# nh2/lz4-frame-conduit

Hardware: AMD Instinct MI355X
Metric: GiB/s end-to-end (compress+decompress), 4 MiB blocks, 1/2/4/8 GPUs vs liblz4 (higher is better)
Workload: dtype u8

## Files before the change

### lz4_frame_conduit_amd/csrc/encode.cuh

```cuda
#pragma once
#include <type_traits>
#include "common.cuh"

namespace lz4f {

constexpr uint32_t MFLIMIT = 12, LASTLIT = 5, MINMATCH = 4;
constexpr uint32_t ENC_POOL_SHORT = 0x200u;

struct ChunkInfo {
    uint32_t nrec;
    uint32_t first_lit;
    uint32_t tail_lit;
    uint32_t body_size;
    uint32_t carry_in;
    uint32_t flags;
    uint64_t out_off;
};

struct EncGeom {
    uint64_t src_size;
    uint64_t first_off;
    uint32_t write_endmark;
    uint32_t block_size;
    uint32_t chunk_size;
    uint32_t chunks_per_block;
    uint32_t n_blocks;
    uint32_t n_chunks;
    uint32_t linked;
    uint32_t block_checksum;
    uint32_t header_size;
    uint8_t  header[20];
    uint32_t max_rec_per_chunk;
    uint64_t rec_pool;
    uint32_t seed_stride;
    uint32_t tiles_per_wg;
    uint32_t e1_solo;
    uint32_t hc_attempts;
    uint32_t hc_lazy;
};

struct EncPlace {
    uint64_t bstart, bend_abs;
    uint64_t cs_abs, ce_abs;
    uint64_t low_abs;
    uint64_t rd_end;
};
__device__ __forceinline__ bool enc_place(const EncGeom& g, uint32_t chunk, EncPlace& pl)
{
    const uint32_t blk = chunk / g.chunks_per_block, cib = chunk % g.chunks_per_block;
    pl.bstart = g.first_off + (uint64_t)blk * g.block_size;
    pl.bend_abs = (pl.bstart + g.block_size < g.src_size) ? pl.bstart + g.block_size : g.src_size;
// ... 39 lines not shown
constexpr uint32_t E1_HASH_LOG = 13;
#ifndef E1_WAVES
#define E1_WAVES 16
#endif
#ifdef E1_DEBUG
#define E1DBG(...) __VA_ARGS__
#else
#define E1DBG(...)
#endif
#define E1_DBG_AT (((uint64_t)gridDim.x) * (2 * E1_NSLICE * E1_REC_PER_SLICE))
struct alignas(16) E1Shared {
    uint16_t table[1u << E1_HASH_LOG];
    uint8_t  tags[1u << E1_HASH_LOG];
    uint32_t s_end[2][E1_NSLICE];
    uint8_t  s_n[2][E1_NSLICE];
    uint32_t next, cov;
    uint32_t first;
    uint32_t cur[16];
    uint32_t pieces[2];
    uint32_t mode, hits;
    uint32_t tail_d[2];
    uint32_t idle[64];
    alignas(16) uint8_t ring[E1_RING + 16];
};
static_assert(sizeof(E1Shared) <= 163840, "one workgroup per CU");
static_assert(64 * E1_WAVES >= E1_NSLICE, "a thread per slice when the lists are merged");
#ifndef E1_GRAB
#define E1_GRAB 8
#endif
#ifndef E1_GRAB_D
#define E1_GRAB_D 1
#endif
#ifndef E1_DENSE_PASS
#define E1_DENSE_PASS 1
#endif
#ifndef E1_V2
// ... 31 lines not shown
#endif
#ifndef E1_STEP_HIT
#define E1_STEP_HIT 1
#endif
constexpr uint32_t E1_GRAB_SPARSE = E1_GRAB, E1_GRAB_DENSE = E1_GRAB_D, E1_PROBE_SLICES = 16, E1_DENSE_HITS = 24;
static_assert((E1_GRAB_SPARSE & (E1_GRAB_SPARSE - 1u)) == 0, "a long helping's size is a power of two: its claims are aligned by masking");

struct __attribute__((aligned(4))) e1_w2 { uint32_t a, b; };
struct __attribute__((aligned(4))) e1_w3 { uint32_t a, b, c; };
__device__ __forceinline__ uint32_t e1_ld32(const uint8_t* ring, uint32_t pos)
{
    const uint32_t i = pos & E1_RMASK;
    const e1_w2 w = *(const e1_w2*)(ring + (i & ~3u));
    return __builtin_amdgcn_alignbyte(w.b, w.a, i & 3u);
}
__device__ __forceinline__ uint64_t e1_ld64(const uint8_t* ring, uint32_t pos)
{
    const uint32_t i = pos & E1_RMASK;
    const e1_w3 w = *(const e1_w3*)(ring + (i & ~3u));
    return (uint64_t)__builtin_amdgcn_alignbyte(w.b, w.a, i & 3u) | ((uint64_t)__builtin_amdgcn_alignbyte(w.c, w.b, i & 3u) << 32);
}
#if E1_V7
static_assert(E1_ROWS >= 1 && E1_ROWS <= 8, "rows per round");
constexpr uint32_t E1_ROW_BYTES = 4 * 64, E1_ROUND_BYTES = E1_ROWS * E1_ROW_BYTES;
struct e1_rows { e1_w2 s1[E1_ROWS], s2[E1_ROWS]; };
__device__ __forceinline__ e1_rows e1_rows_ld(const uint8_t* ring, uint32_t base, uint32_t d, uint32_t lane)
{
    e1_rows w;
#pragma unroll
    for (uint32_t r = 0; r < E1_ROWS; r++) {
// ... 63 lines not shown
    t = (uint32_t)__builtin_amdgcn_update_dpp((int)v, (int)v, 0x112 , 0xf, 0xf, false); v = t < v ? t : v;
    t = (uint32_t)__builtin_amdgcn_update_dpp((int)v, (int)v, 0x114 , 0xf, 0xf, false); v = t < v ? t : v;
    t = (uint32_t)__builtin_amdgcn_update_dpp((int)v, (int)v, 0x118 , 0xf, 0xf, false); v = t < v ? t : v;
    return (uint32_t)__builtin_amdgcn_readlane((int)v, 15);
}
__device__ __forceinline__ uint32_t wave_excl_scan_max(uint32_t v)
{
    const uint32_t lane = lane_id();
    uint32_t incl = v;
#pragma unroll
    for (int sft = 1; sft < 64; sft <<= 1) { const uint32_t t = __shfl_up(incl, sft); if ((int)lane >= sft) incl = t > incl ? t : incl; }
    const uint32_t ex = __shfl_up(incl, 1);
    return lane == 0 ? 0u : ex;
}
constexpr uint32_t E1_PIECE_LOG = 12, E1_NPIECE = E1_TILE >> E1_PIECE_LOG;
__device__ __forceinline__ void e1_dma_piece(E1Shared& sh, const uint8_t* __restrict__ src, uint64_t org, uint32_t nts, uint32_t pc)
{
    const uint32_t lane = lane_id();
    const uint32_t ring0 = (uint32_t)(uintptr_t)(lptr_t)sh.ring;
#pragma unroll
    for (uint32_t q = 0; q < 4; q++) {
        const uint32_t at = nts + (pc << E1_PIECE_LOG) + q * 1024u;
        const uint8_t* gsrc = src + (org + at + lane * 16u);
        const uint32_t ldst = uni(ring0 + (at & E1_RMASK));
        uint32_t keep;
        asm volatile("s_mov_b32 %0, m0\n\ts_mov_b32 m0, %2\n\ts_nop 0\n\tglobal_load_lds_dwordx4 %1, off\n\ts_mov_b32 m0, %0" : "=&s"(keep) : "v"(gsrc), "s"(ldst) : "memory");
    }
}

__device__ __forceinline__ void e1_fill(E1Shared& sh, const uint8_t* __restrict__ src, uint64_t org, uint32_t a, uint32_t b, uint32_t tid)
// ... 142 lines not shown
                        le = st + ml;
                    }
                    cur = nx2;
                }
                const uint32_t e = (sj < nslice) ? s_end[sj] : 0u; cov = e > cov ? e : cov;
            }
        }
        ChunkInfo* ci = info + c;
        if (lane == 0) {
            if (room) { ci->nrec = ktot; ci->first_lit = tile_first; ci->tail_lit = te - kmax; ci->body_size = btot; }
            else      { ci->nrec = 0; ci->first_lit = 0; ci->tail_lit = te - ts; ci->body_size = 0; }
            sh.mode = (uint64_t)ktot * 64 > (uint64_t)(te - ts) ? 2u : 1u;
        }
    };

    if (tid == 0) { sh.mode = 0; sh.cov = E1_TILE; sh.hits = 0; sh.first = 0; sh.next = E1_ALIGN ? 0 : 1; sh.pieces[0] = 0; sh.pieces[1] = 0; sh.tail_d[0] = 0; sh.tail_d[1] = 0; }
    if (tid < 16) sh.cur[tid] = 0;
    uint32_t mode_tile = 0;
    uint32_t hold = 1;
    bool pend = false;
    uint32_t p_c = 0, p_par = 0, p_ts = 0, p_te = 0, p_bend = 0, p_ns = 0;
    __syncthreads();
    for (uint32_t c = c0; c < c1; c++) {
        const uint32_t k = c - c0;
        const uint32_t ts = E1_TILE * (k + 1), par = k & 1u;
        const uint32_t blk = c / g.chunks_per_block;
        const uint64_t bstart = g.first_off + (uint64_t)blk * g.block_size;
        const uint64_t bend_abs = (bstart + g.block_size < g.src_size) ? bstart + g.block_size : g.src_size;
        const uint64_t cs_abs = s0 + (uint64_t)k * E1_TILE;
        if (cs_abs >= bend_abs) {
            ChunkInfo* ci = info + c;
            if (tid == 0) { ci->nrec = 0; ci->first_lit = 0; ci->tail_lit = 0; ci->body_size = 0; }
            continue;
        }
        const uint32_t tlen = (uint32_t)((bend_abs - cs_abs < E1_TILE) ? bend_abs - cs_abs : E1_TILE);
        const uint32_t te = ts + tlen;
        const uint32_t bend = ts + (uint32_t)(bend_abs - cs_abs);
        const uint32_t blen = (uint32_t)(bend_abs - bstart);
        const uint32_t nslice = (tlen + E1_SLICE - 1) / E1_SLICE;
        uint32_t low = hist0;
// ... 1 lines not shown
        uint64_t* spec_t = spec + (size_t)par * (E1_NSLICE * E1_REC_PER_SLICE);

        uint32_t nlen = 0;
        const uint32_t nts = ts + E1_TILE;
        if (c + 1 < c1) {
            const uint32_t nblk = (c + 1) / g.chunks_per_block;
            const uint64_t nbstart = g.first_off + (uint64_t)nblk * g.block_size;
            const uint64_t nbend = (nbstart + g.block_size < g.src_size) ? nbstart + g.block_size : g.src_size;
            const uint64_t ncs = cs_abs + E1_TILE;
            if (ncs < nbend) nlen = (uint32_t)((nbend - ncs < E1_TILE) ? nbend - ncs : E1_TILE);
        }
        const bool nlen_full = nlen == E1_TILE;

        E1DBG(const unsigned long long q0 = clock64();)
        if (pend && wave == E1_WAVES - 1) {
            *(lane == 0 ? &sh.cur[wave] : &sh.idle[lane]) = 0xFFFFFFFFu;
            merge(p_c, p_par, p_ts, p_te, p_bend, p_ns);
        }

        E1DBG(const unsigned long long q1 = clock64();)
        const uint32_t end_lim = (te < bend - LASTLIT) ? te : bend - LASTLIT;
        E1DBG(uint32_t dq = 0; unsigned long long a_deq = 0, a_probe = 0, a_hit = 0, n_step = 0, n_hit = 0, n_deq = 0;)
        bool fresh = true;
        E1DBG(unsigned long long z0 = 0;)
#if E1_V5
        const uint32_t lim_t = (!(g.e1_solo & 2u) && blen >= MFLIMIT + 1) ? ((te - MINMATCH < bend - MFLIMIT) ? te - MINMATCH : bend - MFLIMIT) : 0u;
        const bool tile_plain = !(E1_ALIGN && mode_tile == 1u && !(g.e1_solo & 1u));
        bool plain = tile_plain || hold;
#endif
        auto release = [&](const uint32_t si, const uint32_t grab) __attribute__((always_inline)) {
            if (nlen_full && (si & 31u) < grab) {
                uint32_t mn = lane < E1_WAVES ? __hip_atomic_load(&sh.cur[lane], __ATOMIC_RELAXED, __HIP_MEMORY_SCOPE_WORKGROUP) : 0xFFFFFFFFu;
                mn = wave_min16(mn);
                uint32_t ok_p = mn == 0xFFFFFFFFu ? 0u : (mn * E1_SLICE) >> E1_PIECE_LOG;
                if (ok_p > E1_NPIECE) ok_p = E1_NPIECE;
                const uint32_t had = uni(atomicMax(lane == 0 ? &sh.pieces[par] : &sh.idle[lane], ok_p));
                for (uint32_t pc = had; pc < ok_p; pc++) e1_dma_piece(sh, src, org, ts + E1_TILE, pc);
            }
        };
        auto helping = [&](const uint32_t si, uint32_t ip, const uint32_t mode, const uint32_t grab, const bool opener) __attribute__((always_inline)) {
            const uint32_t cs = ts + si * E1_SLICE;
            uint64_t* myrec = spec_t + si * E1_REC_PER_SLICE;
            E1DBG(a_deq += clock64() - z0;)
            uint32_t nrec = 0, anchor = cs;
            if (ip < cs) ip = cs;
#if E1_V5
            {
                uint32_t last_start = cs + grab * E1_SLICE - 1u;
                if (lim_t < last_start) last_start = lim_t;
#else
            const uint32_t ce = (cs + grab * E1_SLICE < te) ? cs + grab * E1_SLICE : te;
            if (!(g.e1_solo & 2u) && blen >= MFLIMIT + 1 && ip + MINMATCH <= te && ip + MFLIMIT <= bend && ip < ce) {
                uint32_t last_start = ce - 1;
                if (te - MINMATCH < last_start) last_start = te - MINMATCH;
                if (bend - MFLIMIT < last_start) last_start = bend - MFLIMIT;
#endif
                const uint32_t floor_b = ip;
                uint32_t step = (E1_STEP0 > 1 && mode == 1 && !opener) ? (uint32_t)E1_STEP0 : 1u, two = opener ? 0u : 1u;
                E1DBG(uint32_t it = 0;)
                while (ip <= last_start) {
                    E1DBG(if (++it > 100000) { if (lane == 0) { atomicAdd((unsigned long long*)&scratch[E1_DBG_AT + 1], 1ull); scratch[E1_DBG_AT + 8] = ((uint64_t)ip << 32) | last_start; scratch[E1_DBG_AT + 9] = ((uint64_t)step << 32) | si; } break; })
                    E1DBG(const unsigned long long z1 = clock64(); n_step++;)
                    const uint32_t ipB = ip + WAVE * step, stepB = step + 1;
                    const uint32_t pA = ip + lane * step, pB = ipB + lane * stepB;
                    const bool actA = pA <= last_start, actB = two && pB <= last_start;
#if E1_V3
                    const uint32_t iA = pA & E1_RMASK, iB = pB & E1_RMASK;
// ... 92 lines not shown
                            const uint32_t pe = dpp_excl_scan_max(is_t ? lane + fl : 0u);
                            const uint32_t before = pe ? ip + pe : anchor;
                            const uint32_t bfloor = pe ? ip + pe : (anchor > floor_b ? anchor : floor_b);
                            uint32_t nb = nbk;
                            if (pA - bfloor < nb) nb = pA - bfloor;
                            if (pA - di - low < nb) nb = pA - di - low;
                            const uint32_t rank = (uint32_t)__builtin_popcountll(taken & ((1ull << lane) - 1ull));
                            if (is_t) myrec[nrec + rank] = pack_rec(pA - nb - before, fl + nb, di);
                            nrec += (uint32_t)__builtin_popcountll(taken);
                            E1DBG(if (blockIdx.x == 0 && lane == 0) { atomicAdd((unsigned long long*)&scratch[E1_DBG_AT + 13], 1ull); atomicAdd((unsigned long long*)&scratch[E1_DBG_AT + 14], (unsigned long long)__builtin_popcountll(taken)); atomicAdd((unsigned long long*)&scratch[E1_DBG_AT + 15], (unsigned long long)(stop_at < WAVE ? stop_at : (endrel > WAVE ? endrel : WAVE))); })
                            anchor = ip + endrel;
                            const uint32_t nrel = stop_at < WAVE ? stop_at : (endrel > WAVE ? endrel : WAVE);
                            const bool ins2 = actA && lane > L && lane < nrel && lane >= pe;
                            *(ins2 ? &sh.table[hA] : (uint16_t*)&sh.idle[lane]) = (uint16_t)pA; *(ins2 ? &sh.tags[hA] : (uint8_t*)&sh.idle[lane]) = (uint8_t)tgA;
                            ip += nrel;
                            atomicMax(lane == 0 ? &sh.cov : &sh.idle[lane], anchor);
                            step = 1; two = 1;
                            E1DBG(a_hit += clock64() - z2;)
                            continue;
                        }
                    }
                    E1DBG(if (blockIdx.x == 0 && lane == 0) { atomicAdd((unsigned long long*)&scratch[E1_DBG_AT + 4 + (inB ? 0 : mode != 2 ? 1 : step != 1 ? 2 : 3)], 1ull); })
                    const uint32_t dsel = inB ? dB : dA;
                    uint32_t mp = (uint32_t)__builtin_amdgcn_readlane(inB ? pB : pA, L);
                    const uint32_t d = (uint32_t)__builtin_amdgcn_readlane(dsel, L);
                    uint32_t room = mp - (anchor > floor_b ? anchor : floor_b); if (mp - d - low < room) room = mp - d - low;
                    uint32_t nb = 0;
                    E1DBG(uint32_t itb = 0;)
#if E1_V4
                    uint32_t fw = 0;
                    {
// ... 21 lines not shown
                    }
#endif
                    for (bool more = nb == WAVE; more;) {
                        E1DBG(if (++itb > 100000) { if (lane == 0) { atomicAdd((unsigned long long*)&scratch[E1_DBG_AT + 2], 1ull); scratch[E1_DBG_AT + 10] = ((uint64_t)room << 32) | nb; } break; })
                        const uint32_t kb = nb + lane + 1;
                        const uint32_t b1 = sh.ring[(mp - kb) & E1_RMASK], b2 = sh.ring[(mp - d - kb) & E1_RMASK];
                        const uint64_t ne = __ballot(b1 != b2 || kb > room);
                        const uint32_t n1 = ne ? (uint32_t)__builtin_ctzll(ne) : WAVE;
                        nb += n1;
                        more = n1 == WAVE;
                    }
                    E1DBG(uint32_t itf = 0;)
                    while (fw >> 31) {
                        fw &= 0x7FFFFFFFu;
                        E1DBG(if (++itf > 100000) { if (lane == 0) { atomicAdd((unsigned long long*)&scratch[E1_DBG_AT + 3], 1ull); scratch[E1_DBG_AT + 11] = ((uint64_t)mp << 32) | fw; scratch[E1_DBG_AT + 12] = ((uint64_t)end_lim << 32) | d; } break; })
#if E1_V7
                        const uint32_t a0 = mp + fw;
                        const e1_rows w = e1_rows_ld(sh.ring, a0, d, lane);
                        const uint32_t n = e1_rows_same(w, a0 & 3u, (a0 - d) & 3u), cap = end_lim - mp;
                        fw += n;
                        fw = (n == E1_ROUND_BYTES && fw < cap) ? (fw | 0x80000000u) : (fw < cap ? fw : cap);
#else
                        const uint32_t a0 = mp + fw + lane * 16;
                        const e1_w5 s1 = e1_ld5(sh.ring, a0), s2 = e1_ld5(sh.ring, a0 - d);
                        uint32_t g0 = e1_same16(s1, s2, a0 & 3u, (a0 - d) & 3u);
                        const int32_t r = (int32_t)(end_lim - a0); g0 = r <= 0 ? 0u : (g0 > (uint32_t)r ? (uint32_t)r : g0);
                        const uint64_t stop = __ballot(g0 < 16);
                        if (stop) { const uint32_t f = (uint32_t)__builtin_ctzll(stop); fw += f * 16 + (uint32_t)__builtin_amdgcn_readlane(g0, f); }
                        else fw = (fw + WAVE * 16) | 0x80000000u;
#endif
                    }
#else
                    for (;;) {
                        E1DBG(if (++itb > 100000) { if (lane == 0) { atomicAdd((unsigned long long*)&scratch[E1_DBG_AT + 2], 1ull); scratch[E1_DBG_AT + 10] = ((uint64_t)room << 32) | nb; } break; })
                        const uint32_t kb = nb + lane + 1;
                        const bool eq = kb <= room && sh.ring[(mp - kb) & E1_RMASK] == sh.ring[(mp - d - kb) & E1_RMASK];
                        const uint64_t ne = __ballot(!eq);
                        const uint32_t n1 = ne ? (uint32_t)__builtin_ctzll(ne) : WAVE;
                        nb += n1;
                        if (n1 < WAVE) break;
                    }
                    uint32_t fw = 0;
                    E1DBG(uint32_t itf = 0;)
                    for (;;) {
                        E1DBG(if (++itf > 100000) { if (lane == 0) { atomicAdd((unsigned long long*)&scratch[E1_DBG_AT + 3], 1ull); scratch[E1_DBG_AT + 11] = ((uint64_t)mp << 32) | fw; scratch[E1_DBG_AT + 12] = ((uint64_t)end_lim << 32) | d; } break; })
                        const uint32_t a0 = mp + fw + lane * 8;
                        uint32_t g0 = 0;
                        if (a0 < end_lim) {
                            const uint64_t x = e1_ld64(sh.ring, a0) ^ e1_ld64(sh.ring, a0 - d);
                            g0 = x ? (uint32_t)(__builtin_ctzll(x) >> 3) : 8u;
                            const uint32_t r = end_lim - a0; if (g0 > r) g0 = r;
                        }
                        const uint64_t stop = __ballot(g0 < 8);
                        if (stop) { const uint32_t f = (uint32_t)__builtin_ctzll(stop); fw += f * 8 + (uint32_t)__builtin_amdgcn_readlane(g0, f); break; }
                        fw += WAVE * 8;
                    }
#endif
                    mp -= nb;
                    const uint32_t mlen = nb + fw;
                    myrec[nrec] = pack_rec(mp - anchor, mlen, d);
                    nrec++;
                    anchor = ip = mp + mlen;
                    step = (E1_STEP_HIT > 1 && mode == 1) ? (uint32_t)E1_STEP_HIT : 1u; two = 1;
                    atomicMax(lane == 0 ? &sh.cov : &sh.idle[lane], ip);
                    if (E1_OPENER == 2) *((lane == 0 && ip == end_lim) ? &sh.tail_d[par] : &sh.idle[lane]) = d;
                    E1DBG(a_hit += clock64() - z2;)
                    if (E1_IP2 && ip >= low + 2 && ip + 2 <= te) { const uint32_t q2 = ip - 2, hv2 = e1_mix(e1_ld32(sh.ring, q2)); *(lane == 0 ? &sh.table[e1_slot(hv2)] : (uint16_t*)&sh.idle[lane]) = (uint16_t)q2; *(lane == 0 ? &sh.tags[e1_slot(hv2)] : (uint8_t*)&sh.idle[lane]) = (uint8_t)e1_tag(hv2); }
                }
            }
            const bool mine_s = lane < grab && si + lane < nslice;
            *(mine_s ? &sh.s_end[par][si + lane] : &sh.idle[lane]) = (lane == 0 && nrec) ? anchor : 0u;
            *(mine_s ? &sh.s_n[par][si + lane] : (uint8_t*)&sh.idle[lane]) = (uint8_t)(lane == 0 ? nrec : 0u);
            if (mode == 0) atomicAdd(lane == 0 ? &sh.hits : &sh.idle[lane], nrec);
            if (opener) *(lane == 0 ? &sh.first : &sh.idle[lane]) = 1u;
        };
        for (;;) {
            if ((g.e1_solo & 1u) && tid >= WAVE) break;
            E1DBG(z0 = clock64(); n_deq++;)
            E1DBG(if (++dq > 100000) { if (lane == 0) atomicAdd((unsigned long long*)&scratch[E1_DBG_AT + 0], 1ull); break; })
#if E1_V5
            if (!plain) {
                const uint32_t a = atomicAdd(lane == 0 ? &sh.next : &sh.idle[lane], E1_GRAB_SPARSE);
                const uint32_t cv = __hip_atomic_load(&sh.cov, __ATOMIC_RELAXED, __HIP_MEMORY_SCOPE_WORKGROUP);
                __builtin_amdgcn_sched_barrier(0);
                const uint32_t si = uni(a);
                if (si >= nslice) { *(lane == 0 ? &sh.cur[wave] : &sh.idle[lane]) = 0xFFFFFFFFu; break; }
                *(lane == 0 ? &sh.cur[wave] : &sh.idle[lane]) = si;
                release(si, E1_GRAB_SPARSE);
                helping(si, uni(cv), 1u, E1_GRAB_SPARSE, false);
                continue;
            }
            plain = tile_plain;
#endif
            uint32_t mode = (g.e1_solo & 1u) ? mode_tile : uni(__hip_atomic_load(&sh.mode, __ATOMIC_RELAXED, __HIP_MEMORY_SCOPE_WORKGROUP));
            const bool opener = fresh && wave == 0 && (!E1_ALIGN || hold);
            uint32_t grab = opener ? 1u : mode == 1 ? E1_GRAB_SPARSE : mode == 2 ? E1_GRAB_DENSE : 1u;
            uint32_t si = 0;
            if (E1_ALIGN && opener) si = uni(atomicAdd(lane == 0 ? &sh.next : &sh.idle[lane], grab));
            if (!opener) {
                if (fresh && E1_OPENER && ((E1_OPENER == 1 && !E1_ALIGN) || hold)) for (uint32_t spin = 0; spin < 4096 && uni(__hip_atomic_load(&sh.first, __ATOMIC_RELAXED, __HIP_MEMORY_SCOPE_WORKGROUP)) == 0; spin++) __builtin_amdgcn_s_sleep(2);
                bool got = false;
#if E1_V6
                if (E1_ALIGN && mode == 1) {
                    uint32_t n = uni(__hip_atomic_load(&sh.next, __ATOMIC_RELAXED, __HIP_MEMORY_SCOPE_WORKGROUP));
                    for (uint32_t t = 0; t < 64 && !got; t++) {
                        const uint32_t tgt = (n & ~(E1_GRAB_SPARSE - 1u)) + E1_GRAB_SPARSE;
                        const uint32_t old = uni(atomicCAS(lane == 0 ? &sh.next : &sh.idle[lane], n, tgt));
                        if (old == n) { got = true; si = n; grab = tgt - n; }
                        n = old;
                    }
                }
#endif
                if (!got) si = uni(atomicAdd(lane == 0 ? &sh.next : &sh.idle[lane], grab));
            }
            fresh = false;
            if (si >= nslice) { *(lane == 0 ? &sh.cur[wave] : &sh.idle[lane]) = 0xFFFFFFFFu; break; }
            *(lane == 0 ? &sh.cur[wave] : &sh.idle[lane]) = si;
            release(si, grab);
            if (mode == 0 && si >= 2 * E1_PROBE_SLICES) {
                mode = uni(__hip_atomic_load(&sh.hits, __ATOMIC_RELAXED, __HIP_MEMORY_SCOPE_WORKGROUP)) > E1_DENSE_HITS ? 2u : 1u;
                *(lane == 0 ? &sh.mode : &sh.idle[lane]) = mode;
                mode_tile = mode;
            }
            helping(si, uni(__hip_atomic_load(&sh.cov, __ATOMIC_RELAXED, __HIP_MEMORY_SCOPE_WORKGROUP)), mode, grab, opener);
        }
        E1DBG(const unsigned long long q2 = clock64();)
        __builtin_amdgcn_s_waitcnt(0);
        __syncthreads();
        mode_tile = uni(__hip_atomic_load(&sh.mode, __ATOMIC_RELAXED, __HIP_MEMORY_SCOPE_WORKGROUP));
        E1DBG(const unsigned long long q3 = clock64();)
        pend = true; p_c = c; p_par = par; p_ts = ts; p_te = te; p_bend = bend; p_ns = nslice;

        if (tid == 0) { sh.tail_d[par ^ 1u] = 0; sh.cov = nts; sh.hits = 0; sh.first = 0; sh.next = E1_ALIGN ? 0 : 1; sh.pieces[par ^ 1u] = 0; }
        if (tid < 16) sh.cur[tid] = 0;
        if (nlen) {
            if (nlen_full) {
                const uint32_t had = sh.pieces[par];
                for (uint32_t pc = had + wave; pc < E1_NPIECE; pc += E1_WAVES) e1_dma_piece(sh, src, org, nts, pc);
                if ((nts & E1_RMASK) == 0 && tid >= 64 && tid < 68) ((uint32_t*)(sh.ring + E1_RING))[tid - 64] = *(const u32_ua*)(src + (org + nts + (tid - 64) * 4u));
            } else e1_fill(sh, src, org, nts, nts + nlen, tid);
        }
        E1DBG(const unsigned long long q4 = clock64();)
        asm volatile("s_waitcnt vmcnt(0)" ::: "memory");
        E1DBG(const unsigned long long q5 = clock64();)
        __syncthreads();
        {
            const uint32_t td = uni(__hip_atomic_load(&sh.tail_d[par], __ATOMIC_RELAXED, __HIP_MEMORY_SCOPE_WORKGROUP));
            hold = (g.e1_solo & 1u) || (td != 0 && nlen >= 4 && uni(e1_ld32(sh.ring, nts)) == uni(e1_ld32(sh.ring, nts - td))) ? 1u : 0u;
        }
        E1DBG(if (blockIdx.x == 0 && lane == 0) { unsigned long long* d = (unsigned long long*)&scratch[E1_DBG_AT + 16 + wave * 8]; d[0] += q1 - q0; d[1] += q2 - q1; d[2] += q3 - q2; d[3] += q4 - q3; d[4] += q5 - q4; d[5] += clock64() - q5; d[6] += 1; unsigned long long* f = (unsigned long long*)&scratch[E1_DBG_AT + 160 + wave * 6]; f[0] += a_deq; f[1] += a_probe; f[2] += a_hit; f[3] += n_deq; f[4] += n_step; f[5] += n_hit; })
    }
    if (pend && wave == E1_WAVES - 1) merge(p_c, p_par, p_ts, p_te, p_bend, p_ns);
}


__device__ __forceinline__ uint32_t layout_block_chunks(ChunkInfo* __restrict__ ci, const uint32_t nch, const uint32_t blen)
{
    const uint32_t lane = lane_id();
    uint32_t carry_run = 0, total = 0;
    for (uint32_t c0 = 0; c0 < nch; c0 += WAVE) {
        const uint32_t c = c0 + lane;
        const bool act = c < nch;
        const uint4 x = act ? *(const uint4*)&ci[c] : uint4{0u, 0u, 0u, 0u};
// ... 538 lines not shown
```

### lz4_frame_conduit_amd/csrc/engine.hip

```cpp
#include <hip/hip_runtime.h>
#include <stdarg.h>
#include <stdio.h>
#include <stdlib.h>
#include <string.h>

#include <algorithm>
#include <mutex>
#include <vector>

#include "engine.hpp"
#include "frame_dev.cuh"
#include "decode_batch.cuh"
#include "encode_batch.cuh"
#include "measure_batch.cuh"
#include "pack_batch.cuh"

using namespace lz4f;

static_assert(sizeof(ChunkInfo) == 32, "chunk info layout");
static_assert(sizeof(BatchFrame) == 80 && sizeof(BatchBlk) == 40, "batch workspace layout");
static_assert(sizeof(BatchCore) == 64 && sizeof(MeasBlk) == 24, "batch measure workspace layout");
static_assert(sizeof(BcFrame) == 72 && sizeof(BcBlk) == 32 && sizeof(BcChunk) == 64, "batch encode workspace layout");

namespace lz4f {
// ... 56 lines not shown
    no_density_probe = on("LZ4F_MI355X_NO_DENSITY_PROBE");
    no_spx = on("LZ4F_MI355X_NO_SPX");
    no_overlap = on("LZ4F_MI355X_NO_OVERLAP");
    no_content_check = on("LZ4F_MI355X_NO_CONTENT_CHECK");
    prof = on("LZ4F_MI355X_PROF");
    e1_sync = on("LZ4F_MI355X_E1_SYNC");
    no_selffeed = on("LZ4F_MI355X_NO_SELFFEED");
    dense_mode = (unsigned)num("LZ4F_MI355X_DENSE_MODE", 0, 2, 0);
    group_kib = (unsigned)num("LZ4F_MI355X_GROUP_KIB", 64, 4096, 0);
    if (group_kib & (group_kib - 1)) group_kib = 0;
    feed_round = (unsigned)num("LZ4F_MI355X_FEED_ROUND", 17, 4096, 0);
    chain_gate = num("LZ4F_MI355X_CHAIN_GATE", 1, (1 << 20) - 1, 0);
    decode_mode = 0; if (const char* v = getenv("LZ4F_MI355X_DECODE")) decode_mode = v[0];
    e1_run = (unsigned)num("LZ4F_MI355X_E1_RUN", 1, 4096, 0);
    e1_solo = 0; if (const char* v = getenv("LZ4F_MI355X_E1_SOLO")) e1_solo = (unsigned)atoi(v);
    if (on("LZ4F_MI355X_DETERMINISTIC")) e1_solo |= 1u;
    wait_ticks = 0; if (const char* v = getenv("LZ4F_MI355X_WAIT_TICKS")) { unsigned long long a = 0; if (sscanf(v, "%llu", &a) == 1) wait_ticks = a; }
    dblk_lds = (unsigned)num("LZ4F_MI355X_DBLK_LDS", 1, 150, 0) << 10;
    recs_per_tile = (unsigned)num("LZ4F_MI355X_RECS_PER_TILE", 1, 16385, 0);
    hc_attempts = (unsigned)num("LZ4F_MI355X_HC_ATTEMPTS", 1, 65536, 0);
    hc_lazy = (unsigned)num("LZ4F_MI355X_HC_LAZY", 1, 2, 0);
    seed = 2; if (const char* v = getenv("LZ4F_MI355X_SEED")) { unsigned a = 0; if (sscanf(v, "%u", &a) == 1 && a >= 1 && a <= 64) seed = a; }
}
namespace lz4f {
size_t new_engine(lz4f_mi355x_engine** out, int device, void* stream, bool borrow)
{
    int n = 0;
    hipError_t e = hipGetDeviceCount(&n);
    if (e != hipSuccess || n <= 0) {
        set_last_error("no usable HIP device (hipGetDeviceCount: %s, count %d): liblz4f_mi355x has no CPU fallback", hipGetErrorString(e), n);
// ... 169 lines not shown
    g.seed_stride = sw.seed;
    const bool hc = j.level >= 3;
    p.finder = hc ? EncodePlan::HASH_CHAIN : ((sw.e1_solo & 1u) && !(sw.e1_solo & 4u)) ? EncodePlan::E1_SOLO : EncodePlan::E1_SHARED;
    if (hc) {
        const HcLevel hl = hc_level(j.level);
        g.hc_attempts = sw.hc_attempts ? sw.hc_attempts : hl.attempts;
        g.hc_lazy = sw.hc_lazy ? sw.hc_lazy : hl.lazy;
    }
    g.rec_pool = rec_pool_records(g.n_chunks, g.max_rec_per_chunk, ((sw.e1_solo & 1u) || hc) ? 16385u : sw.recs_per_tile);
    if (g.n_chunks) {
        uint32_t run = g.n_chunks / cus; run = run < 1 ? 1 : run > 64 ? 64 : run;
        if ((g.n_chunks + run - 1) / run > 1024) run = (g.n_chunks + 1023) / 1024;
        if (sw.e1_run) run = sw.e1_run;
        g.tiles_per_wg = run;
        g.e1_solo = sw.e1_solo;
        p.e1_wgs = (g.n_chunks + run - 1) / run;
        p.e1_scratch_bytes = (size_t)p.e1_wgs * 2 * E1_NSLICE * E1_REC_PER_SLICE * 8 + 2048;
    }
    p.layout_small = g.n_blocks <= LAYOUT_SMALL_BLOCKS && g.n_chunks <= LAYOUT_SMALL_CHUNKS; p.e2_split = g.n_chunks <= 512;
    p.xxh_lane4 = g.n_blocks < XXH_LANE4_BELOW;
    p.inband = inband;
    p.index_cap = inband ? index_capacity(payload, s) + 64 : index_cap;
    p.ixtmp_bytes = inband ? p.index_cap + 64 : 0;
    p.info_bytes = (size_t)(g.n_chunks + 1) * sizeof(ChunkInfo); p.recs_bytes = (size_t)(rec_pool_at(g.n_chunks) + g.rec_pool) * 8;
    p.blk_bytes = (size_t)(g.n_blocks + 1) * 4; p.table_bytes = (size_t)(g.n_blocks + 1) * sizeof(BlockOut);
    p.res_bytes = sizeof(ResultRec) + sizeof(TrailerPlan) + 64;
    return p;
}

#ifdef E1_DEBUG
static void e1_debug_dump(hipStream_t st, const uint8_t* counters)
{
    unsigned long long d[256]; if (hipStreamSynchronize(st) == hipSuccess && hipMemcpy(d, counters, 2048, hipMemcpyDeviceToHost) == hipSuccess) {
                for (int w = 0; w < 16; w += 5) { unsigned long long* x = d + 16 + w * 8; if (x[6]) fprintf(stderr, "E1 wave %d: per tile cycles: merge %llu parse %llu waitB1 %llu dma-issue %llu dma-wait %llu waitB2 %llu (%llu tiles)\n", w, x[0]/x[6], x[1]/x[6], x[2]/x[6], x[3]/x[6], x[4]/x[6], x[5]/x[6], x[6]); unsigned long long* f = d + 160 + w * 6; fprintf(stderr, "   parse: dequeue %llu cycles x %llu, probe step %llu cycles x %llu, hit %llu cycles x %llu (per tile)\n", f[3] ? f[0]/f[3] : 0, f[3]/x[6], f[4] ? f[1]/f[4] : 0, f[4]/x[6], f[5] ? f[2]/f[5] : 0, f[5]/x[6]); }
                fprintf(stderr, "E1 dense passes (workgroup 0): %llu, matches taken %llu, positions advanced %llu; one-match steps because: hit in B %llu, mode not dense %llu, step != 1 %llu, first match long %llu\n", d[13], d[14], d[15], d[4], d[5], d[6], d[7]);
                fprintf(stderr, "E1 debug: bounds hit: dequeue %llu, probe %llu, backward %llu, forward %llu; probe ip/last %llx step/slice %llx; back room/nb %llx; fwd mp/fw %llx end_lim/d %llx\n", d[0], d[1], d[2], d[3], d[8], d[9], d[10], d[11], d[12]); }
}
#endif

size_t lz4f_mi355x_engine::enc_workspaces(const EncodePlan& p, bool own_table)
{
    if (ixtmp.ensure(p.ixtmp_bytes) || res.ensure(p.res_bytes) || info.ensure(p.info_bytes) || recs.ensure(p.recs_bytes) || blk_bytes.ensure(p.blk_bytes) ||
        (own_table && table.ensure(p.table_bytes)) || e1_scratch.ensure(p.e1_scratch_bytes))
        return make_err(LZ4F_ERROR_allocation_failed);
    return 0;
}

size_t lz4f_mi355x_engine::enc_find(const CompressJob& j, const EncodePlan& p)
{
    hipStream_t st = (hipStream_t)stream; const EncGeom& g = p.g;
#ifdef E1_DEBUG
// ... 1037 lines not shown
```

### lz4_frame_conduit_amd/csrc/engine.hpp

```cpp
#pragma once
#include <stddef.h>
#include <stdint.h>
#include <functional>
#include <string>
#include <vector>

#include "../../include/lz4f_mi355x.h"
#include "records.hpp"

namespace lz4f {

inline size_t make_err(int code) { return (size_t)-(ptrdiff_t)code; }
inline bool   is_err(size_t v) { return v > make_err(LZ4F_ERROR_maxCode); }
const char*   err_name(size_t v);
void          set_last_error(const char* fmt, ...);
const char*   last_error();

struct Xxh32State {
    uint32_t total_len, large, v[4], memsize;
    uint8_t  mem[16];
    void reset(uint32_t seed = 0);
    void update(const void* data, size_t len);
    uint32_t digest() const;
};
// ... 41 lines not shown
    lz4f::DevBuf pdbuf;
    lz4f::DevBuf tight;
    lz4f::DevBuf postab;
    lz4f::DevBuf desc, seqcnt;
    lz4f::DevBuf d_in, d_out;
    lz4f::DevBuf bframes, btable;
    lz4f::DevBuf mframes, mtable;
    lz4f::DevBuf pctl;
    lz4f::DevBuf cframes, cblocks, cchunks;
    lz4f::PinBuf h_in, h_out, h_small;
    struct Switches {
        bool no_index, no_selfindex, no_resolve, no_trace, no_doubling, trace_always, no_groups, no_window, serial_walk, no_trailer, no_content_check, no_density_probe, no_spx, no_overlap, prof, e1_sync, no_selffeed;
        unsigned dense_mode;
        unsigned group_kib;
        unsigned feed_round;
        int chain_gate; char decode_mode; unsigned e1_run, e1_solo, seed, dblk_lds, recs_per_tile, hc_attempts, hc_lazy; unsigned long long wait_ticks;
        void read();
    } sw;
    void*  recs_ctl_clean = nullptr;
    size_t ix_seq_cap = 0;
    bool  timing = false;
    void* ev[24] = {nullptr};
    bool  ev_used[12] = {false};
    void  tick(int slot, bool end, void* on_stream = nullptr);
    void* aux_stream = nullptr; void* ev_fork = nullptr; void* ev_join = nullptr;
    bool  aux_ready();
    bool  aux_pending = false;

    struct CompressJob {
        const uint8_t* d_src; uint64_t src_size; uint64_t first_off;
        uint32_t block_size; bool linked; bool block_checksum; bool endmark;
// ... 104 lines not shown
```

Baseline: 794.0.

## Replace end-of-tile barrier with per-piece landed bits so next tile starts early

```diff
diff --git a/lz4_frame_conduit_amd/csrc/encode.cuh b/lz4_frame_conduit_amd/csrc/encode.cuh
--- a/lz4_frame_conduit_amd/csrc/encode.cuh
+++ b/lz4_frame_conduit_amd/csrc/encode.cuh
@@ -35,6 +35,7 @@
     uint32_t seed_stride;
     uint32_t tiles_per_wg;
     uint32_t e1_solo;
+    uint32_t e1_close;
     uint32_t hc_attempts;
     uint32_t hc_lazy;
 };
@@ -104,12 +105,14 @@
     uint8_t  tags[1u << E1_HASH_LOG];
     uint32_t s_end[2][E1_NSLICE];
     uint8_t  s_n[2][E1_NSLICE];
-    uint32_t next, cov;
-    uint32_t first;
-    uint32_t cur[16];
-    uint32_t pieces[2];
-    uint32_t mode, hits;
-    uint32_t tail_d[2];
+    uint32_t next[2], cov[2];
+    uint32_t first[2];
+    uint32_t cur[2][16];
+    uint32_t hits[2];
+    uint32_t landed[2];
+    uint32_t pieces[4];
+    uint32_t mode;
+    uint32_t tail_d[4];
     uint32_t idle[64];
     alignas(16) uint8_t ring[E1_RING + 16];
 };
@@ -171,6 +174,12 @@
     const e1_w2 w = *(const e1_w2*)(ring + (i & ~3u));
     return __builtin_amdgcn_alignbyte(w.b, w.a, i & 3u);
 }
+__device__ __forceinline__ uint32_t e1_ld32_wrap(const uint8_t* ring, uint32_t pos)
+{
+    const uint32_t i = pos & E1_RMASK, i0 = i & ~3u;
+    const uint32_t a = *(const uint32_t*)(ring + i0), b = *(const uint32_t*)(ring + ((i0 + 4u) & E1_RMASK));
+    return __builtin_amdgcn_alignbyte(b, a, i & 3u);
+}
 __device__ __forceinline__ uint64_t e1_ld64(const uint8_t* ring, uint32_t pos)
 {
     const uint32_t i = pos & E1_RMASK;
@@ -264,6 +273,31 @@
     return lane == 0 ? 0u : ex;
 }
 constexpr uint32_t E1_PIECE_LOG = 12, E1_NPIECE = E1_TILE >> E1_PIECE_LOG;
+#if E1_V4 && E1_V7
+constexpr uint32_t E1_FWD_BYTES = E1_ROUND_BYTES;
+#elif E1_V4
+constexpr uint32_t E1_FWD_BYTES = 64 * 16;
+#else
+constexpr uint32_t E1_FWD_BYTES = 64 * 8;
+#endif
+constexpr uint32_t E1_REACH = E1_FWD_BYTES + 16, E1_TAIL_BIT = 1u << E1_NPIECE, E1_LANDED_ALL = (1u << (E1_NPIECE + 1)) - 1u;
+#ifndef E1_LAND_BUDGET
+#define E1_LAND_BUDGET 4096
+#endif
+__device__ __forceinline__ uint32_t e1_need(uint32_t ts, uint32_t end, uint32_t tail)
+{
+    return ((2u << ((end - 1u - ts) >> E1_PIECE_LOG)) - 1u) | tail;
+}
+__device__ __forceinline__ bool e1_wait_landed(const uint32_t* word, uint32_t need, uint32_t have)
+{
+    for (uint32_t spin = 0; (have & need) != need; spin++) {
+        if (spin >= E1_LAND_BUDGET) return false;
+        __builtin_amdgcn_s_sleep(2);
+        have = uni(__hip_atomic_load(word, __ATOMIC_RELAXED, __HIP_MEMORY_SCOPE_WORKGROUP));
+    }
+    asm volatile("" ::: "memory");
+    return true;
+}
 __device__ __forceinline__ void e1_dma_piece(E1Shared& sh, const uint8_t* __restrict__ src, uint64_t org, uint32_t nts, uint32_t pc)
 {
     const uint32_t lane = lane_id();
@@ -436,8 +470,10 @@
         }
     };
 
-    if (tid == 0) { sh.mode = 0; sh.cov = E1_TILE; sh.hits = 0; sh.first = 0; sh.next = E1_ALIGN ? 0 : 1; sh.pieces[0] = 0; sh.pieces[1] = 0; sh.tail_d[0] = 0; sh.tail_d[1] = 0; }
-    if (tid < 16) sh.cur[tid] = 0;
+    if (tid < 2) { sh.cov[tid] = E1_TILE * (tid + 1); sh.hits[tid] = 0; sh.first[tid] = 0; sh.next[tid] = E1_ALIGN ? 0 : 1; sh.landed[tid] = tid ? 0u : E1_LANDED_ALL; }
+    if (tid < 4) { sh.pieces[tid] = 0; sh.tail_d[tid] = 0; }
+    if (tid == 0) sh.mode = 0;
+    if (tid < 32) sh.cur[tid >> 4][tid & 15u] = 0;
     uint32_t mode_tile = 0;
     uint32_t hold = 1;
     bool pend = false;
@@ -445,7 +481,9 @@
     __syncthreads();
     for (uint32_t c = c0; c < c1; c++) {
         const uint32_t k = c - c0;
-        const uint32_t ts = E1_TILE * (k + 1), par = k & 1u;
+        const uint32_t ts = E1_TILE * (k + 1), par = k & 1u, k4 = k & 3u;
+        const uint32_t tail_bit = (ts & E1_RMASK) == 0 ? E1_TAIL_BIT : 0u;
+        const uint32_t full_bits = (E1_TAIL_BIT - 1u) | tail_bit;
         const uint32_t blk = c / g.chunks_per_block;
         const uint64_t bstart = g.first_off + (uint64_t)blk * g.block_size;
         const uint64_t bend_abs = (bstart + g.block_size < g.src_size) ? bstart + g.block_size : g.src_size;
@@ -477,7 +515,7 @@
 
         E1DBG(const unsigned long long q0 = clock64();)
         if (pend && wave == E1_WAVES - 1) {
-            *(lane == 0 ? &sh.cur[wave] : &sh.idle[lane]) = 0xFFFFFFFFu;
+            *(lane == 0 ? &sh.cur[par][wave] : &sh.idle[lane]) = 0xFFFFFFFFu;
             merge(p_c, p_par, p_ts, p_te, p_bend, p_ns);
         }
 
@@ -489,21 +527,29 @@
 #if E1_V5
         const uint32_t lim_t = (!(g.e1_solo & 2u) && blen >= MFLIMIT + 1) ? ((te - MINMATCH < bend - MFLIMIT) ? te - MINMATCH : bend - MFLIMIT) : 0u;
         const bool tile_plain = !(E1_ALIGN && mode_tile == 1u && !(g.e1_solo & 1u));
+        const bool tile_guard = mode_tile == 1u || (g.e1_solo & 1u);
         bool plain = tile_plain || hold;
 #endif
         auto release = [&](const uint32_t si, const uint32_t grab) __attribute__((always_inline)) {
             if (nlen_full && (si & 31u) < grab) {
-                uint32_t mn = lane < E1_WAVES ? __hip_atomic_load(&sh.cur[lane], __ATOMIC_RELAXED, __HIP_MEMORY_SCOPE_WORKGROUP) : 0xFFFFFFFFu;
+                uint32_t mn = lane < E1_WAVES ? __hip_atomic_load(&sh.cur[par][lane], __ATOMIC_RELAXED, __HIP_MEMORY_SCOPE_WORKGROUP) : 0xFFFFFFFFu;
                 mn = wave_min16(mn);
                 uint32_t ok_p = mn == 0xFFFFFFFFu ? 0u : (mn * E1_SLICE) >> E1_PIECE_LOG;
                 if (ok_p > E1_NPIECE) ok_p = E1_NPIECE;
-                const uint32_t had = uni(atomicMax(lane == 0 ? &sh.pieces[par] : &sh.idle[lane], ok_p));
+                const uint32_t had = uni(atomicMax(lane == 0 ? &sh.pieces[k4] : &sh.idle[lane], ok_p));
                 for (uint32_t pc = had; pc < ok_p; pc++) e1_dma_piece(sh, src, org, ts + E1_TILE, pc);
             }
         };
-        auto helping = [&](const uint32_t si, uint32_t ip, const uint32_t mode, const uint32_t grab, const bool opener) __attribute__((always_inline)) {
+        auto helping = [&](const uint32_t si, uint32_t ip, const uint32_t mode, const uint32_t grab, const bool opener, const uint32_t lw) __attribute__((always_inline)) {
             const uint32_t cs = ts + si * E1_SLICE;
             uint64_t* myrec = spec_t + si * E1_REC_PER_SLICE;
+            bool in_ring = true;
+            if ((lw & full_bits) != full_bits) {
+                const uint32_t gend = cs + grab * E1_SLICE + E1_REACH;
+                in_ring = e1_wait_landed(&sh.landed[par], E1_LAND_BUDGET ? e1_need(ts, gend < te ? gend : te, tail_bit) : full_bits, lw);
+            }
+            asm volatile("" ::: "memory");
+            E1DBG(if (!in_ring && lane == 0) atomicAdd((unsigned long long*)&scratch[E1_DBG_AT + 144], 1ull);)
             E1DBG(a_deq += clock64() - z0;)
             uint32_t nrec = 0, anchor = cs;
             if (ip < cs) ip = cs;
@@ -511,9 +557,10 @@
             {
                 uint32_t last_start = cs + grab * E1_SLICE - 1u;
                 if (lim_t < last_start) last_start = lim_t;
+                if (!in_ring) last_start = 0;
 #else
             const uint32_t ce = (cs + grab * E1_SLICE < te) ? cs + grab * E1_SLICE : te;
-            if (!(g.e1_solo & 2u) && blen >= MFLIMIT + 1 && ip + MINMATCH <= te && ip + MFLIMIT <= bend && ip < ce) {
+            if (in_ring && !(g.e1_solo & 2u) && blen >= MFLIMIT + 1 && ip + MINMATCH <= te && ip + MFLIMIT <= bend && ip < ce) {
                 uint32_t last_start = ce - 1;
                 if (te - MINMATCH < last_start) last_start = te - MINMATCH;
                 if (bend - MFLIMIT < last_start) last_start = bend - MFLIMIT;
@@ -636,7 +683,7 @@
                             const bool ins2 = actA && lane > L && lane < nrel && lane >= pe;
                             *(ins2 ? &sh.table[hA] : (uint16_t*)&sh.idle[lane]) = (uint16_t)pA; *(ins2 ? &sh.tags[hA] : (uint8_t*)&sh.idle[lane]) = (uint8_t)tgA;
                             ip += nrel;
-                            atomicMax(lane == 0 ? &sh.cov : &sh.idle[lane], anchor);
+                            atomicMax(lane == 0 ? &sh.cov[par] : &sh.idle[lane], anchor);
                             step = 1; two = 1;
                             E1DBG(a_hit += clock64() - z2;)
                             continue;
@@ -688,6 +735,14 @@
                     while (fw >> 31) {
                         fw &= 0x7FFFFFFFu;
                         E1DBG(if (++itf > 100000) { if (lane == 0) { atomicAdd((unsigned long long*)&scratch[E1_DBG_AT + 3], 1ull); scratch[E1_DBG_AT + 11] = ((uint64_t)mp << 32) | fw; scratch[E1_DBG_AT + 12] = ((uint64_t)end_lim << 32) | d; } break; })
+                        {
+                            const uint32_t fe = mp + fw + E1_REACH, lf = uni(__hip_atomic_load(&sh.landed[par], __ATOMIC_RELAXED, __HIP_MEMORY_SCOPE_WORKGROUP));
+                            if ((lf & full_bits) != full_bits && !e1_wait_landed(&sh.landed[par], E1_LAND_BUDGET ? e1_need(ts, fe < te ? fe : te, tail_bit) : full_bits, lf)) {
+                                E1DBG(if (lane == 0) atomicAdd((unsigned long long*)&scratch[E1_DBG_AT + 145], 1ull);)
+                                break;
+                            }
+                            asm volatile("" ::: "memory");
+                        }
 #if E1_V7
                         const uint32_t a0 = mp + fw;
                         const e1_rows w = e1_rows_ld(sh.ring, a0, d, lane);
@@ -718,6 +773,14 @@
                     E1DBG(uint32_t itf = 0;)
                     for (;;) {
                         E1DBG(if (++itf > 100000) { if (lane == 0) { atomicAdd((unsigned long long*)&scratch[E1_DBG_AT + 3], 1ull); scratch[E1_DBG_AT + 11] = ((uint64_t)mp << 32) | fw; scratch[E1_DBG_AT + 12] = ((uint64_t)end_lim << 32) | d; } break; })
+                        if (fw) {
+                            const uint32_t fe = mp + fw + E1_REACH, lf = uni(__hip_atomic_load(&sh.landed[par], __ATOMIC_RELAXED, __HIP_MEMORY_SCOPE_WORKGROUP));
+                            if ((lf & full_bits) != full_bits && !e1_wait_landed(&sh.landed[par], E1_LAND_BUDGET ? e1_need(ts, fe < te ? fe : te, tail_bit) : full_bits, lf)) {
+                                E1DBG(if (lane == 0) atomicAdd((unsigned long long*)&scratch[E1_DBG_AT + 145], 1ull);)
+                                break;
+                            }
+                            asm volatile("" ::: "memory");
+                        }
                         const uint32_t a0 = mp + fw + lane * 8;
                         uint32_t g0 = 0;
                         if (a0 < end_lim) {
@@ -736,8 +799,8 @@
                     nrec++;
                     anchor = ip = mp + mlen;
                     step = (E1_STEP_HIT > 1 && mode == 1) ? (uint32_t)E1_STEP_HIT : 1u; two = 1;
-                    atomicMax(lane == 0 ? &sh.cov : &sh.idle[lane], ip);
-                    if (E1_OPENER == 2) *((lane == 0 && ip == end_lim) ? &sh.tail_d[par] : &sh.idle[lane]) = d;
+                    atomicMax(lane == 0 ? &sh.cov[par] : &sh.idle[lane], ip);
+                    if (E1_OPENER == 2) *((lane == 0 && ip == end_lim) ? &sh.tail_d[k4] : &sh.idle[lane]) = d;
                     E1DBG(a_hit += clock64() - z2;)
                     if (E1_IP2 && ip >= low + 2 && ip + 2 <= te) { const uint32_t q2 = ip - 2, hv2 = e1_mix(e1_ld32(sh.ring, q2)); *(lane == 0 ? &sh.table[e1_slot(hv2)] : (uint16_t*)&sh.idle[lane]) = (uint16_t)q2; *(lane == 0 ? &sh.tags[e1_slot(hv2)] : (uint8_t*)&sh.idle[lane]) = (uint8_t)e1_tag(hv2); }
                 }
@@ -745,23 +808,27 @@
             const bool mine_s = lane < grab && si + lane < nslice;
             *(mine_s ? &sh.s_end[par][si + lane] : &sh.idle[lane]) = (lane == 0 && nrec) ? anchor : 0u;
             *(mine_s ? &sh.s_n[par][si + lane] : (uint8_t*)&sh.idle[lane]) = (uint8_t)(lane == 0 ? nrec : 0u);
-            if (mode == 0) atomicAdd(lane == 0 ? &sh.hits : &sh.idle[lane], nrec);
-            if (opener) *(lane == 0 ? &sh.first : &sh.idle[lane]) = 1u;
+            if (mode == 0) atomicAdd(lane == 0 ? &sh.hits[par] : &sh.idle[lane], nrec);
+            if (opener) *(lane == 0 ? &sh.first[par] : &sh.idle[lane]) = 1u;
         };
         for (;;) {
-            if ((g.e1_solo & 1u) && tid >= WAVE) break;
+            if ((g.e1_solo & 1u) && tid >= WAVE) {
+                *(lane == 0 ? &sh.cur[par][wave] : &sh.idle[lane]) = 0xFFFFFFFFu;
+                break;
+            }
             E1DBG(z0 = clock64(); n_deq++;)
             E1DBG(if (++dq > 100000) { if (lane == 0) atomicAdd((unsigned long long*)&scratch[E1_DBG_AT + 0], 1ull); break; })
 #if E1_V5
             if (!plain) {
-                const uint32_t a = atomicAdd(lane == 0 ? &sh.next : &sh.idle[lane], E1_GRAB_SPARSE);
-                const uint32_t cv = __hip_atomic_load(&sh.cov, __ATOMIC_RELAXED, __HIP_MEMORY_SCOPE_WORKGROUP);
+                const uint32_t a = atomicAdd(lane == 0 ? &sh.next[par] : &sh.idle[lane], E1_GRAB_SPARSE);
+                const uint32_t cv = __hip_atomic_load(&sh.cov[par], __ATOMIC_RELAXED, __HIP_MEMORY_SCOPE_WORKGROUP);
+                const uint32_t lw = __hip_atomic_load(&sh.landed[par], __ATOMIC_RELAXED, __HIP_MEMORY_SCOPE_WORKGROUP);
                 __builtin_amdgcn_sched_barrier(0);
                 const uint32_t si = uni(a);
-                if (si >= nslice) { *(lane == 0 ? &sh.cur[wave] : &sh.idle[lane]) = 0xFFFFFFFFu; break; }
-                *(lane == 0 ? &sh.cur[wave] : &sh.idle[lane]) = si;
+                if (si >= nslice) { *(lane == 0 ? &sh.cur[par][wave] : &sh.idle[lane]) = 0xFFFFFFFFu; break; }
+                *(lane == 0 ? &sh.cur[par][wave] : &sh.idle[lane]) = si;
                 release(si, E1_GRAB_SPARSE);
-                helping(si, uni(cv), 1u, E1_GRAB_SPARSE, false);
+                helping(si, uni(cv), 1u, E1_GRAB_SPARSE, false, uni(lw));
                 continue;
             }
             plain = tile_plain;
@@ -770,33 +837,39 @@
             const bool opener = fresh && wave == 0 && (!E1_ALIGN || hold);
             uint32_t grab = opener ? 1u : mode == 1 ? E1_GRAB_SPARSE : mode == 2 ? E1_GRAB_DENSE : 1u;
             uint32_t si = 0;
-            if (E1_ALIGN && opener) si = uni(atomicAdd(lane == 0 ? &sh.next : &sh.idle[lane], grab));
+            if (E1_ALIGN && opener) si = uni(atomicAdd(lane == 0 ? &sh.next[par] : &sh.idle[lane], grab));
             if (!opener) {
-                if (fresh && E1_OPENER && ((E1_OPENER == 1 && !E1_ALIGN) || hold)) for (uint32_t spin = 0; spin < 4096 && uni(__hip_atomic_load(&sh.first, __ATOMIC_RELAXED, __HIP_MEMORY_SCOPE_WORKGROUP)) == 0; spin++) __builtin_amdgcn_s_sleep(2);
+                if (fresh && E1_OPENER && ((E1_OPENER == 1 && !E1_ALIGN) || hold)) for (uint32_t spin = 0; spin < 4096 && uni(__hip_atomic_load(&sh.first[par], __ATOMIC_RELAXED, __HIP_MEMORY_SCOPE_WORKGROUP)) == 0; spin++) __builtin_amdgcn_s_sleep(2);
                 bool got = false;
 #if E1_V6
                 if (E1_ALIGN && mode == 1) {
-                    uint32_t n = uni(__hip_atomic_load(&sh.next, __ATOMIC_RELAXED, __HIP_MEMORY_SCOPE_WORKGROUP));
+                    uint32_t n = uni(__hip_atomic_load(&sh.next[par], __ATOMIC_RELAXED, __HIP_MEMORY_SCOPE_WORKGROUP));
                     for (uint32_t t = 0; t < 64 && !got; t++) {
                         const uint32_t tgt = (n & ~(E1_GRAB_SPARSE - 1u)) + E1_GRAB_SPARSE;
-                        const uint32_t old = uni(atomicCAS(lane == 0 ? &sh.next : &sh.idle[lane], n, tgt));
+                        const uint32_t old = uni(atomicCAS(lane == 0 ? &sh.next[par] : &sh.idle[lane], n, tgt));
                         if (old == n) { got = true; si = n; grab = tgt - n; }
                         n = old;
                     }
                 }
 #endif
-                if (!got) si = uni(atomicAdd(lane == 0 ? &sh.next : &sh.idle[lane], grab));
+                if (!got) si = uni(atomicAdd(lane == 0 ? &sh.next[par] : &sh.idle[lane], grab));
             }
             fresh = false;
-            if (si >= nslice) { *(lane == 0 ? &sh.cur[wave] : &sh.idle[lane]) = 0xFFFFFFFFu; break; }
-            *(lane == 0 ? &sh.cur[wave] : &sh.idle[lane]) = si;
+            if (si >= nslice) { *(lane == 0 ? &sh.cur[par][wave] : &sh.idle[lane]) = 0xFFFFFFFFu; break; }
+            *(lane == 0 ? &sh.cur[par][wave] : &sh.idle[lane]) = si;
             release(si, grab);
             if (mode == 0 && si >= 2 * E1_PROBE_SLICES) {
-                mode = uni(__hip_atomic_load(&sh.hits, __ATOMIC_RELAXED, __HIP_MEMORY_SCOPE_WORKGROUP)) > E1_DENSE_HITS ? 2u : 1u;
+                mode = uni(__hip_atomic_load(&sh.hits[par], __ATOMIC_RELAXED, __HIP_MEMORY_SCOPE_WORKGROUP)) > E1_DENSE_HITS ? 2u : 1u;
                 *(lane == 0 ? &sh.mode : &sh.idle[lane]) = mode;
                 mode_tile = mode;
             }
-            helping(si, uni(__hip_atomic_load(&sh.cov, __ATOMIC_RELAXED, __HIP_MEMORY_SCOPE_WORKGROUP)), mode, grab, opener);
+            {
+                const uint32_t cv = __hip_atomic_load(&sh.cov[par], __ATOMIC_RELAXED, __HIP_MEMORY_SCOPE_WORKGROUP);
+                uint32_t lw = E1_LANDED_ALL;
+                if (tile_guard) lw = __hip_atomic_load(&sh.landed[par], __ATOMIC_RELAXED, __HIP_MEMORY_SCOPE_WORKGROUP);
+                const uint32_t lwu = uni(lw);
+                helping(si, uni(cv), mode, grab, opener, lwu);
+            }
         }
         E1DBG(const unsigned long long q2 = clock64();)
         __builtin_amdgcn_s_waitcnt(0);
@@ -805,22 +878,42 @@
         E1DBG(const unsigned long long q3 = clock64();)
         pend = true; p_c = c; p_par = par; p_ts = ts; p_te = te; p_bend = bend; p_ns = nslice;
 
-        if (tid == 0) { sh.tail_d[par ^ 1u] = 0; sh.cov = nts; sh.hits = 0; sh.first = 0; sh.next = E1_ALIGN ? 0 : 1; sh.pieces[par ^ 1u] = 0; }
-        if (tid < 16) sh.cur[tid] = 0;
-        if (nlen) {
-            if (nlen_full) {
-                const uint32_t had = sh.pieces[par];
-                for (uint32_t pc = had + wave; pc < E1_NPIECE; pc += E1_WAVES) e1_dma_piece(sh, src, org, nts, pc);
-                if ((nts & E1_RMASK) == 0 && tid >= 64 && tid < 68) ((uint32_t*)(sh.ring + E1_RING))[tid - 64] = *(const u32_ua*)(src + (org + nts + (tid - 64) * 4u));
-            } else e1_fill(sh, src, org, nts, nts + nlen, tid);
-        }
-        E1DBG(const unsigned long long q4 = clock64();)
-        asm volatile("s_waitcnt vmcnt(0)" ::: "memory");
-        E1DBG(const unsigned long long q5 = clock64();)
-        __syncthreads();
+        if (tid == 0) { sh.tail_d[k4 ^ 2u] = 0; sh.pieces[k4 ^ 2u] = 0; sh.cov[par] = nts + E1_TILE; sh.hits[par] = 0; sh.first[par] = 0; sh.next[par] = E1_ALIGN ? 0 : 1; sh.landed[par] = 0; }
+        if (tid < 16) sh.cur[par][tid] = 0;
+        const uint32_t had = nlen_full ? uni(__hip_atomic_load(&sh.pieces[k4], __ATOMIC_RELAXED, __HIP_MEMORY_SCOPE_WORKGROUP)) : 0u;
+        E1DBG(unsigned long long q4, q5;)
+        if (g.e1_close != 2u && nlen_full && had >= 1u && (mode_tile == 1u || (g.e1_solo & 1u))) {
+            const uint32_t pc = had + wave;
+            if (pc < E1_NPIECE) e1_dma_piece(sh, src, org, nts, pc);
+            uint32_t mine = (1u << had) - 1u;
+            if ((nts & E1_RMASK) == 0 && wave == 1) {
+                if (lane < 4) ((uint32_t*)(sh.ring + E1_RING))[lane] = ((const uint32_t*)sh.ring)[lane];
+                mine |= E1_TAIL_BIT;
+                asm volatile("s_waitcnt lgkmcnt(0)" ::: "memory");
+            }
+            atomicOr(lane == 0 ? &sh.landed[par ^ 1u] : &sh.idle[lane], mine);
+            E1DBG(q4 = clock64();)
+            if (pc < E1_NPIECE) {
+                asm volatile("s_waitcnt vmcnt(0)" ::: "memory");
+                atomicOr(lane == 0 ? &sh.landed[par ^ 1u] : &sh.idle[lane], 1u << pc);
+            }
+            E1DBG(q5 = clock64();)
+        } else {
+            if (nlen) {
+                if (nlen_full) {
+                    for (uint32_t pc = had + wave; pc < E1_NPIECE; pc += E1_WAVES) e1_dma_piece(sh, src, org, nts, pc);
+                    if ((nts & E1_RMASK) == 0 && tid >= 64 && tid < 68) ((uint32_t*)(sh.ring + E1_RING))[tid - 64] = *(const u32_ua*)(src + (org + nts + (tid - 64) * 4u));
+                } else e1_fill(sh, src, org, nts, nts + nlen, tid);
+            }
+            if (tid == 0) sh.landed[par ^ 1u] = E1_LANDED_ALL;
+            E1DBG(q4 = clock64();)
+            asm volatile("s_waitcnt vmcnt(0)" ::: "memory");
+            E1DBG(q5 = clock64();)
+            __syncthreads();
+        }
         {
-            const uint32_t td = uni(__hip_atomic_load(&sh.tail_d[par], __ATOMIC_RELAXED, __HIP_MEMORY_SCOPE_WORKGROUP));
-            hold = (g.e1_solo & 1u) || (td != 0 && nlen >= 4 && uni(e1_ld32(sh.ring, nts)) == uni(e1_ld32(sh.ring, nts - td))) ? 1u : 0u;
+            const uint32_t td = uni(__hip_atomic_load(&sh.tail_d[k4], __ATOMIC_RELAXED, __HIP_MEMORY_SCOPE_WORKGROUP));
+            hold = (g.e1_solo & 1u) || (td != 0 && nlen >= 4 && uni(e1_ld32_wrap(sh.ring, nts)) == uni(e1_ld32_wrap(sh.ring, nts - td))) ? 1u : 0u;
         }
         E1DBG(if (blockIdx.x == 0 && lane == 0) { unsigned long long* d = (unsigned long long*)&scratch[E1_DBG_AT + 16 + wave * 8]; d[0] += q1 - q0; d[1] += q2 - q1; d[2] += q3 - q2; d[3] += q4 - q3; d[4] += q5 - q4; d[5] += clock64() - q5; d[6] += 1; unsigned long long* f = (unsigned long long*)&scratch[E1_DBG_AT + 160 + wave * 6]; f[0] += a_deq; f[1] += a_probe; f[2] += a_hit; f[3] += n_deq; f[4] += n_step; f[5] += n_hit; })
     }
diff --git a/lz4_frame_conduit_amd/csrc/engine.hip b/lz4_frame_conduit_amd/csrc/engine.hip
--- a/lz4_frame_conduit_amd/csrc/engine.hip
+++ b/lz4_frame_conduit_amd/csrc/engine.hip
@@ -94,6 +94,7 @@
     decode_mode = 0; if (const char* v = getenv("LZ4F_MI355X_DECODE")) decode_mode = v[0];
     e1_run = (unsigned)num("LZ4F_MI355X_E1_RUN", 1, 4096, 0);
     e1_solo = 0; if (const char* v = getenv("LZ4F_MI355X_E1_SOLO")) e1_solo = (unsigned)atoi(v);
+    e1_close = (unsigned)num("LZ4F_MI355X_E1_CLOSE", 1, 2, 1);
     if (on("LZ4F_MI355X_DETERMINISTIC")) e1_solo |= 1u;
     wait_ticks = 0; if (const char* v = getenv("LZ4F_MI355X_WAIT_TICKS")) { unsigned long long a = 0; if (sscanf(v, "%llu", &a) == 1) wait_ticks = a; }
     dblk_lds = (unsigned)num("LZ4F_MI355X_DBLK_LDS", 1, 150, 0) << 10;
@@ -293,6 +294,7 @@
         if (sw.e1_run) run = sw.e1_run;
         g.tiles_per_wg = run;
         g.e1_solo = sw.e1_solo;
+        g.e1_close = sw.e1_close;
         p.e1_wgs = (g.n_chunks + run - 1) / run;
         p.e1_scratch_bytes = (size_t)p.e1_wgs * 2 * E1_NSLICE * E1_REC_PER_SLICE * 8 + 2048;
     }
@@ -311,9 +313,9 @@
 static void e1_debug_dump(hipStream_t st, const uint8_t* counters)
 {
     unsigned long long d[256]; if (hipStreamSynchronize(st) == hipSuccess && hipMemcpy(d, counters, 2048, hipMemcpyDeviceToHost) == hipSuccess) {
-                for (int w = 0; w < 16; w += 5) { unsigned long long* x = d + 16 + w * 8; if (x[6]) fprintf(stderr, "E1 wave %d: per tile cycles: merge %llu parse %llu waitB1 %llu dma-issue %llu dma-wait %llu waitB2 %llu (%llu tiles)\n", w, x[0]/x[6], x[1]/x[6], x[2]/x[6], x[3]/x[6], x[4]/x[6], x[5]/x[6], x[6]); unsigned long long* f = d + 160 + w * 6; fprintf(stderr, "   parse: dequeue %llu cycles x %llu, probe step %llu cycles x %llu, hit %llu cycles x %llu (per tile)\n", f[3] ? f[0]/f[3] : 0, f[3]/x[6], f[4] ? f[1]/f[4] : 0, f[4]/x[6], f[5] ? f[2]/f[5] : 0, f[5]/x[6]); }
+                for (int w = 0; w < 16; w += 5) { unsigned long long* x = d + 16 + w * 8; if (x[6]) fprintf(stderr, "E1 wave %d: per tile cycles: merge %llu parse %llu waitB1 %llu dma-issue %llu dma-wait %llu waitB2|publish %llu (%llu tiles)\n", w, x[0]/x[6], x[1]/x[6], x[2]/x[6], x[3]/x[6], x[4]/x[6], x[5]/x[6], x[6]); unsigned long long* f = d + 160 + w * 6; fprintf(stderr, "   parse: dequeue %llu cycles x %llu, probe step %llu cycles x %llu, hit %llu cycles x %llu (per tile)\n", f[3] ? f[0]/f[3] : 0, f[3]/x[6], f[4] ? f[1]/f[4] : 0, f[4]/x[6], f[5] ? f[2]/f[5] : 0, f[5]/x[6]); }
                 fprintf(stderr, "E1 dense passes (workgroup 0): %llu, matches taken %llu, positions advanced %llu; one-match steps because: hit in B %llu, mode not dense %llu, step != 1 %llu, first match long %llu\n", d[13], d[14], d[15], d[4], d[5], d[6], d[7]);
-                fprintf(stderr, "E1 debug: bounds hit: dequeue %llu, probe %llu, backward %llu, forward %llu; probe ip/last %llx step/slice %llx; back room/nb %llx; fwd mp/fw %llx end_lim/d %llx\n", d[0], d[1], d[2], d[3], d[8], d[9], d[10], d[11], d[12]); }
+                fprintf(stderr, "E1 debug: bounds hit: dequeue %llu, probe %llu, backward %llu, forward %llu; probe ip/last %llx step/slice %llx; back room/nb %llx; fwd mp/fw %llx end_lim/d %llx; helpings given up for bytes that had not landed %llu, forward measures cut there %llu\n", d[0], d[1], d[2], d[3], d[8], d[9], d[10], d[11], d[12], d[144], d[145]); }
 }
 #endif
 
diff --git a/lz4_frame_conduit_amd/csrc/engine.hpp b/lz4_frame_conduit_amd/csrc/engine.hpp
--- a/lz4_frame_conduit_amd/csrc/engine.hpp
+++ b/lz4_frame_conduit_amd/csrc/engine.hpp
@@ -79,7 +79,7 @@
         unsigned dense_mode;
         unsigned group_kib;
         unsigned feed_round;
-        int chain_gate; char decode_mode; unsigned e1_run, e1_solo, seed, dblk_lds, recs_per_tile, hc_attempts, hc_lazy; unsigned long long wait_ticks;
+        int chain_gate; char decode_mode; unsigned e1_run, e1_solo, e1_close, seed, dblk_lds, recs_per_tile, hc_attempts, hc_lazy; unsigned long long wait_ticks;
         void read();
     } sw;
     void*  recs_ctl_clean = nullptr;
```

New measurement: 820.1 (median of 6 runs). +3.3%, better.
